# 331658260/Drone-YOLO

Measured on AMD Instinct MI355X. Metric: images/sec @640x640 Drone-YOLO-s, higher is better.
Workload: dtype fp16; 1 GPU; Drone-YOLO-s (yolov8s-p2-repvgg.yaml, nc=10) inference 640x640: layout+forward+decode+NMS, inputs resident in HBM; fp16 storage / fp32 accumulate (BASELINE config 2 names bf16: bf16 storage fails the IoU >= 0.999 bar - 0.995 - so the headline runs the 16-bit format that meets it; same MFMA rate, same bytes); batch_per_gpu=256, global_batch=256, parallelism=batch-split x1, no collective, hipgraph=True, streams=2, max_det=300

## Files before the change

drone-yolo_amd/csrc/conv3x3_hreg.hip:

```cpp
#include "common_hip.h"
#include "conv_args.h"

namespace DY_NS {


struct HregArgs {
  const void* x;
  const void* w;
  const float* bias;
  const void* res;
  void* y;
  int N, H, W, Cin, ldx, Cout, ldy, ldres, act;
  int tilesX, tilesY, tilesN, nSpatial;
  unsigned x_bytes, y_bytes, r_bytes;
  double* stats;
  const float* bnb_mean;
  const float* bnb_rstd;
  const float* bnb_gamma;
  const float* bnb_beta;
  int bnb_act;
  int dbg;
};

#ifdef DYOLO_ABLATE
#define HR_DBG(bit) (p.dbg & (bit))
#else
#define HR_DBG(bit) 0
#endif

constexpr int kHrTH = 8, kHrTW = 16, kHrHH = 10, kHrHW = 24;
constexpr int kHrStage = 16 * 1024;
constexpr int kHrStages = 3;

template <typename T, int NCH, bool RES, bool STATS = false, bool BNB = false, int BW = 3>
__global__ __launch_bounds__(256, NCH <= 2 ? (BNB ? BW : 3) : 2) void conv3x3_hreg_kernel(const HregArgs p) {
  static_assert(!(BNB && (RES || STATS)), "BNB: its own mode");
  constexpr bool SLOTS = STATS || BNB, RLOAD = RES || BNB;
  constexpr int EPC = Elem<T>::EPC;
  __shared__ __attribute__((aligned(1024))) unsigned char smem[kHrStages * kHrStage];
  __shared__ f32x4 bnc[BNB ? 64 : 1];
  const int tid = threadIdx.x, lane = tid & 63, wave = tid >> 6;
  const int lq = lane >> 4, lr = lane & 15;
  const __amdgpu_buffer_rsrc_t yrs = __builtin_amdgcn_make_buffer_rsrc(p.y, 0, p.y_bytes, 0x00020000);
  const __amdgpu_buffer_rsrc_t rrs = __builtin_amdgcn_make_buffer_rsrc(const_cast<void*>(p.res ? p.res : p.y), 0, p.res ? p.r_bytes : 0u, 0x00020000);

  const int G = (int)gridDim.x;
  const int logical = ((int)blockIdx.x & 7) * (G >> 3) + ((int)blockIdx.x >> 3);
  const int nt = logical % p.tilesN;
  const int sb = logical / p.tilesN, Gs = G / p.tilesN;
  const int myTiles = sb < p.nSpatial ? (p.nSpatial - sb + Gs - 1) / Gs : 0;
  if constexpr (SLOTS) {
    if (blockIdx.x == 0)
      for (int i = tid; i < 2 * p.Cout; i += 256) p.stats[i] = 0.0;
    if (myTiles <= 0 && tid < 128) {
      const int co = nt * 64 + (tid & 63);
      if (co < p.Cout) p.stats[(size_t)(1 + sb) * 2 * p.Cout + (tid >> 6) * p.Cout + co] = 0.0;
    }
  }
  if (myTiles <= 0) return;
  const int nItems = myTiles * NCH;

  u32x4 wreg[NCH][9];
  {
    const u32x4* wg = reinterpret_cast<const u32x4*>(p.w) + (size_t)nt * NCH * 9 * 4 * 64;
#pragma unroll
    for (int c = 0; c < NCH; ++c)
#pragma unroll
      for (int t = 0; t < 9; ++t) wreg[c][t] = wg[((c * 9 + t) * 4 + wave) * 64 + lane];
  }
  const f32x4 bias4 = *reinterpret_cast<const f32x4*>(p.bias + nt * 64 + wave * 16 + lq * 4);

  constexpr int NDMA = 4;
  constexpr unsigned kOob = 0xfffffff0u;
  const unsigned pre = (unsigned)((p.W + 1) * p.ldx) * 2u;
  const __amdgpu_buffer_rsrc_t xrs = __builtin_amdgcn_make_buffer_rsrc(const_cast<char*>(reinterpret_cast<const char*>(p.x)) - pre, 0, p.x_bytes + pre, 0x00020000);
  unsigned rel[NDMA];
  int hyx[NDMA];
#pragma unroll
  for (int k = 0; k < NDMA; ++k) {
    const int s = (k * 4 + wave) * 64 + lane;
    const int pix = s >> 2, part = s & 3;
    const int hy = pix / kHrHW, hx = pix - hy * kHrHW;
    const bool dead = hx >= kHrTW + 2 || hy >= kHrHH;
    rel[k] = dead ? kOob : (unsigned)((hy * p.W + hx) * p.ldx + (part ^ ((hx >> 1) & 3)) * EPC) * 2u;
    hyx[k] = hy | (hx << 8);
  }
  unsigned voff[NDMA];
  unsigned l_base = 0;
  int l_tile = sb, l_chunk = 0, l_item = 0;
  auto setup_tile = [&](int tile) {
    const int tx = tile % p.tilesX;
    const int r = tile / p.tilesX;
    const int ty = r % p.tilesY, n = r / p.tilesY;
    const int y0 = ty * kHrTH, x0 = tx * kHrTW;
    l_base = (unsigned)(((n * p.H + y0) * p.W + x0) * p.ldx) * 2u;
    const bool interior = y0 > 0 && y0 + kHrTH + 1 <= p.H && x0 > 0 && x0 + kHrTW + 1 <= p.W;
    if (interior) {
#pragma unroll
      for (int k = 0; k < NDMA; ++k) voff[k] = rel[k];
    } else {
#pragma unroll
      for (int k = 0; k < NDMA; ++k) {
        const int gy = y0 - 1 + (hyx[k] & 255), gx = x0 - 1 + (hyx[k] >> 8);
        voff[k] = ((unsigned)gy < (unsigned)p.H && (unsigned)gx < (unsigned)p.W) ? rel[k] : kOob;
      }
    }
  };
  auto issue_dma = [&](int stage) {
    unsigned char* sa = smem + stage * kHrStage;
    const bool live = l_item < nItems && !(HR_DBG(4) && l_item >= 2);
    if (live) {
      const unsigned soff = l_base + (unsigned)l_chunk * (4u * EPC * (unsigned)sizeof(T));
#pragma unroll
      for (int k = 0; k < NDMA; ++k)
        __builtin_amdgcn_raw_ptr_buffer_load_lds(xrs, (__attribute__((address_space(3))) void*)(sa + (k * 4 + wave) * 1024), 16, (int)voff[k], (int)soff, 0, 0);
      ++l_item;
      if (++l_chunk == NCH) {
        l_chunk = 0;
        l_tile += Gs;
        if (l_item < nItems) setup_tile(l_tile);
      }
    } else {
#pragma unroll
      for (int k = 0; k < NDMA; ++k)
        __builtin_amdgcn_raw_ptr_buffer_load_lds(xrs, (__attribute__((address_space(3))) void*)(sa + (k * 4 + wave) * 1024), 16, (int)kOob, 0, 0, 0);
    }
  };

  int lane_base[3];
#pragma unroll
  for (int q = 0; q < 3; ++q) lane_base[q] = (lr + q) * 64 + ((lq ^ (((lr + q) >> 1) & 3)) * 16);

  f32x4 acc[kHrTH];
#pragma unroll
  for (int o = 0; o < kHrTH; ++o) acc[o] = bias4;

  auto compute = [&](int stg, int c) {
    const unsigned char* sa = smem + stg * kHrStage;
#pragma unroll
    for (int iy = 0; iy < kHrHH; ++iy) {
      u32x4 a[3];
#pragma unroll
      for (int q = 0; q < 3; ++q) a[q] = *reinterpret_cast<const u32x4*>(sa + lane_base[q] + (HR_DBG(8) ? 0 : iy * (kHrHW * 64)));
#pragma unroll
      for (int r = 0; r < 3; ++r) {
        const int o = iy - r;
        if (o >= 0 && o < kHrTH) {
#pragma unroll
          for (int q = 0; q < 3; ++q) {
            if (HR_DBG(2)) asm volatile("" ::"v"(a[q]));
            else acc[o] = Elem<T>::mma(wreg[c][r * 3 + q], a[q], acc[o]);
          }
        }
      }
    }
  };

  typedef __attribute__((ext_vector_type(4))) T t4;
  u32x4 rl[kHrTH / 2];
  auto load_residual = [&](int tile) {
    const int tx = tile % p.tilesX;
    const int r = tile / p.tilesX;
    const int ty = r % p.tilesY, n = r / p.tilesY;
    const int xx = tx * kHrTW + lr;
    const int co16 = nt * 64 + wave * 16 + (lq >> 1) * 8;
#pragma unroll
    for (int o = 0; o < kHrTH; o += 2) {
      const int yy = ty * kHrTH + o + (lq & 1);
      const bool ok = yy < p.H && xx < p.W;
      const unsigned off = ok ? (unsigned)((((size_t)(n * p.H + yy) * p.W + xx) * (size_t)p.ldres + co16) * sizeof(T)) : 0xfffffff0u;
      rl[o / 2] = __builtin_amdgcn_raw_buffer_load_b128(rrs, off, 0, 0);
    }
  };
  unsigned lane_out[kHrTH / 2];
  {
    const int co16 = nt * 64 + wave * 16 + (lq >> 1) * 8;
#pragma unroll
    for (int o = 0; o < kHrTH; o += 2) lane_out[o / 2] = (unsigned)(((o + (lq & 1)) * p.W + lr) * p.ldy + co16) * (unsigned)sizeof(T);
  }
  float st_sum[4] = {0.f, 0.f, 0.f, 0.f}, st_sq[4] = {0.f, 0.f, 0.f, 0.f};
  if constexpr (BNB) {
    if (tid < 64) {
      const int co = nt * 64 + tid;
      const float mu = p.bnb_mean[co], rs = p.bnb_rstd[co], gr = p.bnb_gamma[co] * rs;
      bnc[tid] = f32x4{rs, -mu * rs, gr, p.bnb_beta[co] - gr * mu};
    }
    asm volatile("s_waitcnt lgkmcnt(0)" ::: "memory");
  }
  auto epilogue = [&](int tile) {
    const int tx = tile % p.tilesX;
    const int r = tile / p.tilesX;
    const int ty = r % p.tilesY, n = r / p.tilesY;
    const int y0 = ty * kHrTH, x0 = tx * kHrTW;
    const unsigned out_base = (unsigned)(((n * p.H + y0) * p.W + x0) * p.ldy) * (unsigned)sizeof(T);
    const bool whole = y0 + kHrTH <= p.H && x0 + kHrTW <= p.W;
    u32x2 pk[kHrTH];
#pragma unroll
    for (int o = 0; o < kHrTH; ++o) {
      float v[4] = {acc[o][0], acc[o][1], acc[o][2], acc[o][3]};
      if (p.act == DY_ACT_SILU) {
#pragma unroll
        for (int e = 0; e < 4; ++e) v[e] = silu_f32(v[e]);
      }
      if constexpr (RES) {
        const auto sx = __builtin_amdgcn_permlane16_swap(rl[o / 2][0], rl[o / 2][2], false, false);
        const auto sy = __builtin_amdgcn_permlane16_swap(rl[o / 2][1], rl[o / 2][3], false, false);
        const t4 rr = __builtin_bit_cast(t4, u32x2{sx[o & 1], sy[o & 1]});
#pragma unroll
        for (int e = 0; e < 4; ++e) v[e] += Elem<T>::to_f32(rr[e]);
      }
      t4 ov;
#pragma unroll
      for (int e = 0; e < 4; ++e) ov[e] = Elem<T>::from_f32(v[e]);
      if constexpr (STATS) {
        if (whole || (y0 + o < p.H && x0 + lr < p.W)) {
#pragma unroll
          for (int e = 0; e < 4; ++e) {
            const float f = Elem<T>::to_f32(ov[e]);
            st_sum[e] += f, st_sq[e] += f * f;
          }
        }
      }
      if constexpr (BNB) {
        const auto sx = __builtin_amdgcn_permlane16_swap(rl[o / 2][0], rl[o / 2][2], false, false);
        const auto sy = __builtin_amdgcn_permlane16_swap(rl[o / 2][1], rl[o / 2][3], false, false);
        const t4 zz = __builtin_bit_cast(t4, u32x2{sx[o & 1], sy[o & 1]});
        if (whole || (y0 + o < p.H && x0 + lr < p.W)) {
#pragma unroll
          for (int e = 0; e < 4; ++e) {
            const f32x4 k = bnc[wave * 16 + lq * 4 + e];
            const float zf = Elem<T>::to_f32(zz[e]);
            const float xh = zf * k[0] + k[1];
            float du = Elem<T>::to_f32(ov[e]);
            if (p.bnb_act == DY_ACT_SILU) {
              const float u = zf * k[2] + k[3];
              const float sg = __builtin_amdgcn_rcpf(1.0f + __builtin_amdgcn_exp2f(u * -1.4426950408889634f));
              du *= sg * (1.0f + u * (1.0f - sg));
            }
            st_sum[e] += du, st_sq[e] += du * xh;
          }
        }
      }
      pk[o] = __builtin_bit_cast(u32x2, ov);
      acc[o] = bias4;
    }
#pragma unroll
    for (int o = 0; o < kHrTH; o += 2) {
      const auto sx = __builtin_amdgcn_permlane16_swap(pk[o][0], pk[o + 1][0], false, false);
      const auto sy = __builtin_amdgcn_permlane16_swap(pk[o][1], pk[o + 1][1], false, false);
      unsigned off = lane_out[o / 2];
      if (!whole) off = (y0 + o + (lq & 1) < p.H && x0 + lr < p.W) ? off : kOob;
      __builtin_amdgcn_raw_buffer_store_b128(u32x4{sx[0], sy[0], sx[1], sy[1]}, yrs, HR_DBG(1) ? kOob : off, (int)out_base, 0);
    }
  };

  setup_tile(l_tile);
  issue_dma(0);
  issue_dma(1 % kHrStages);
  asm volatile("s_waitcnt vmcnt(0)" ::: "memory");
  __builtin_amdgcn_s_barrier();
  int c_tile = sb;
  int stage = 0;
  for (int it = 0; it < nItems; it += NCH) {
#pragma unroll
    for (int c = 0; c < NCH; ++c) {
      if constexpr (RLOAD) {
        if (c == NCH - 1) load_residual(c_tile);
      }
      issue_dma(stage + 2 >= kHrStages ? stage + 2 - kHrStages : stage + 2);
      compute(stage, c);
      if (c == NCH - 1) {
        epilogue(c_tile);
        c_tile += Gs;
      }
      asm volatile("s_waitcnt vmcnt(0)" ::: "memory");
      __builtin_amdgcn_s_barrier();
      stage = stage + 1 == kHrStages ? 0 : stage + 1;
    }
  }
  if constexpr (SLOTS) {
#pragma unroll
    for (int e = 0; e < 4; ++e) {
      float a = st_sum[e], b = st_sq[e];
#pragma unroll
      for (int m = 1; m < 16; m <<= 1) a += __shfl_xor(a, m, 64), b += __shfl_xor(b, m, 64);
      const int co = nt * 64 + wave * 16 + lq * 4 + e;
      if (lr == 0 && co < p.Cout) {
        double* slot = p.stats + (size_t)(1 + sb) * 2 * p.Cout;
        slot[co] = (double)a, slot[p.Cout + co] = (double)b;
      }
    }
  }
}

constexpr int kH2TH = 4, kH2TW = 16, kH2HH = 9, kH2Pitch = 40, kH2PlaneB = 24;
constexpr int kH2Stage = 24 * 1024;

template <typename T, int NCH, bool STATS = false>
__global__ __launch_bounds__(256, 2) void conv3x3_hreg_s2_kernel(const HregArgs p) {
  constexpr int EPC = Elem<T>::EPC;
  __shared__ __attribute__((aligned(1024))) unsigned char smem[kHrStages * kH2Stage];
  const int tid = threadIdx.x, lane = tid & 63, wave = tid >> 6;
  const int lq = lane >> 4, lr = lane & 15;
  const __amdgpu_buffer_rsrc_t yrs = __builtin_amdgcn_make_buffer_rsrc(p.y, 0, p.y_bytes, 0x00020000);
  const int Ho = (p.H - 1) / 2 + 1, Wo = (p.W - 1) / 2 + 1;

  const int G = (int)gridDim.x;
  const int logical = ((int)blockIdx.x & 7) * (G >> 3) + ((int)blockIdx.x >> 3);
  const int nt = logical % p.tilesN;
  const int sb = logical / p.tilesN, Gs = G / p.tilesN;
  const int myTiles = sb < p.nSpatial ? (p.nSpatial - sb + Gs - 1) / Gs : 0;
  if constexpr (STATS) {
    if (blockIdx.x == 0)
      for (int i = tid; i < 2 * p.Cout; i += 256) p.stats[i] = 0.0;
    if (myTiles <= 0 && tid < 128) {
      const int co = nt * 64 + (tid & 63);
      if (co < p.Cout) p.stats[(size_t)(1 + sb) * 2 * p.Cout + (tid >> 6) * p.Cout + co] = 0.0;
    }
  }
  if (myTiles <= 0) return;
  const int nItems = myTiles * NCH;

  u32x4 wreg[NCH][9];
  {
    const u32x4* wg = reinterpret_cast<const u32x4*>(p.w) + (size_t)nt * NCH * 9 * 4 * 64;
#pragma unroll
    for (int c = 0; c < NCH; ++c)
#pragma unroll
      for (int t = 0; t < 9; ++t) wreg[c][t] = wg[((c * 9 + t) * 4 + wave) * 64 + lane];
  }
  const f32x4 bias4 = *reinterpret_cast<const f32x4*>(p.bias + nt * 64 + wave * 16 + lq * 4);

  constexpr int NDMA = 6;
  constexpr unsigned kOob = 0xfffffff0u;
  const unsigned pre = (unsigned)((p.W + 1) * p.ldx) * 2u;
  const __amdgpu_buffer_rsrc_t xrs = __builtin_amdgcn_make_buffer_rsrc(const_cast<char*>(reinterpret_cast<const char*>(p.x)) - pre, 0, p.x_bytes + pre, 0x00020000);
  unsigned rel[NDMA];
  int hyx[NDMA];
#pragma unroll
  for (int k = 0; k < NDMA; ++k) {
    const int s = (k * 4 + wave) * 64 + lane;
    const int slot = s >> 2, part = s & 3;
    const int hy = slot / kH2Pitch, c = slot - hy * kH2Pitch;
    const bool planeB = c >= kH2PlaneB;
    const int ci = planeB ? c - kH2PlaneB : c;
    const int hx = planeB ? 2 * ci + 1 : 2 * ci;
    const bool dead = hy >= kH2HH || hx > 2 * kH2TW;
    rel[k] = dead ? kOob : (unsigned)((hy * p.W + hx) * p.ldx + (part ^ ((ci >> 1) & 3)) * EPC) * 2u;
    hyx[k] = hy | (hx << 8);
  }
  unsigned voff[NDMA];
  unsigned l_base = 0;
  int l_tile = sb, l_chunk = 0, l_item = 0;
  auto setup_tile = [&](int tile) {
    const int tx = tile % p.tilesX;
    const int r = tile / p.tilesX;
    const int ty = r % p.tilesY, n = r / p.tilesY;
    const int y0 = 2 * ty * kH2TH, x0 = 2 * tx * kH2TW;
    l_base = (unsigned)(((n * p.H + y0) * p.W + x0) * p.ldx) * 2u;
    const bool interior = y0 > 0 && y0 - 1 + kH2HH <= p.H && x0 > 0 && x0 + 2 * kH2TW <= p.W;
    if (interior) {
#pragma unroll
      for (int k = 0; k < NDMA; ++k) voff[k] = rel[k];
    } else {
#pragma unroll
      for (int k = 0; k < NDMA; ++k) {
        const int gy = y0 - 1 + (hyx[k] & 255), gx = x0 - 1 + (hyx[k] >> 8);
        voff[k] = ((unsigned)gy < (unsigned)p.H && (unsigned)gx < (unsigned)p.W) ? rel[k] : kOob;
      }
    }
  };
  auto issue_dma = [&](int stage) {
    unsigned char* sa = smem + stage * kH2Stage;
    const bool live = l_item < nItems;
    if (live) {
      const unsigned soff = l_base + (unsigned)l_chunk * (4u * EPC * (unsigned)sizeof(T));
#pragma unroll
      for (int k = 0; k < NDMA; ++k)
        __builtin_amdgcn_raw_ptr_buffer_load_lds(xrs, (__attribute__((address_space(3))) void*)(sa + (k * 4 + wave) * 1024), 16, (int)voff[k], (int)soff, 0, 0);
      ++l_item;
      if (++l_chunk == NCH) {
        l_chunk = 0;
        l_tile += Gs;
        if (l_item < nItems) setup_tile(l_tile);
      }
    } else {
#pragma unroll
      for (int k = 0; k < NDMA; ++k)
        __builtin_amdgcn_raw_ptr_buffer_load_lds(xrs, (__attribute__((address_space(3))) void*)(sa + (k * 4 + wave) * 1024), 16, (int)kOob, 0, 0, 0);
    }
  };

  int lane_base[3];
  lane_base[0] = lr * 64 + ((lq ^ ((lr >> 1) & 3)) * 16);
  lane_base[1] = (kH2PlaneB + lr) * 64 + ((lq ^ ((lr >> 1) & 3)) * 16);
  lane_base[2] = (lr + 1) * 64 + ((lq ^ (((lr + 1) >> 1) & 3)) * 16);

  f32x4 acc[kH2TH];
#pragma unroll
  for (int o = 0; o < kH2TH; ++o) acc[o] = bias4;

  auto compute = [&](int stg, int c) {
    const unsigned char* sa = smem + stg * kH2Stage;
#pragma unroll
    for (int iy = 0; iy < kH2HH; ++iy) {
      u32x4 a[3];
#pragma unroll
      for (int q = 0; q < 3; ++q) a[q] = *reinterpret_cast<const u32x4*>(sa + lane_base[q] + iy * (kH2Pitch * 64));
#pragma unroll
      for (int r = 0; r < 3; ++r) {
        if ((iy - r) % 2 == 0) {
          const int o = (iy - r) / 2;
          if (iy - r >= 0 && o < kH2TH) {
#pragma unroll
            for (int q = 0; q < 3; ++q) acc[o] = Elem<T>::mma(wreg[c][r * 3 + q], a[q], acc[o]);
          }
        }
      }
    }
  };

  typedef __attribute__((ext_vector_type(4))) T t4;
  unsigned lane_out[kH2TH / 2];
  {
    const int co16 = nt * 64 + wave * 16 + (lq >> 1) * 8;
#pragma unroll
    for (int o = 0; o < kH2TH; o += 2) lane_out[o / 2] = (unsigned)(((o + (lq & 1)) * Wo + lr) * p.ldy + co16) * (unsigned)sizeof(T);
  }
  float st_sum[4] = {0.f, 0.f, 0.f, 0.f}, st_sq[4] = {0.f, 0.f, 0.f, 0.f};
  auto epilogue = [&](int tile) {
    const int tx = tile % p.tilesX;
    const int r = tile / p.tilesX;
    const int ty = r % p.tilesY, n = r / p.tilesY;
    const int y0 = ty * kH2TH, x0 = tx * kH2TW;
    const unsigned out_base = (unsigned)(((n * Ho + y0) * Wo + x0) * p.ldy) * (unsigned)sizeof(T);
    const bool whole = y0 + kH2TH <= Ho && x0 + kH2TW <= Wo;
    u32x2 pk[kH2TH];
#pragma unroll
    for (int o = 0; o < kH2TH; ++o) {
      float v[4] = {acc[o][0], acc[o][1], acc[o][2], acc[o][3]};
      if (p.act == DY_ACT_SILU) {
#pragma unroll
        for (int e = 0; e < 4; ++e) v[e] = silu_f32(v[e]);
      }
      t4 ov;
#pragma unroll
      for (int e = 0; e < 4; ++e) ov[e] = Elem<T>::from_f32(v[e]);
      pk[o] = __builtin_bit_cast(u32x2, ov);
      if constexpr (STATS) {
        if (whole || (y0 + o < Ho && x0 + lr < Wo)) {
#pragma unroll
          for (int e = 0; e < 4; ++e) {
            const float f = Elem<T>::to_f32(ov[e]);
            st_sum[e] += f, st_sq[e] += f * f;
          }
        }
      }
      acc[o] = bias4;
    }
#pragma unroll
    for (int o = 0; o < kH2TH; o += 2) {
      const auto sx = __builtin_amdgcn_permlane16_swap(pk[o][0], pk[o + 1][0], false, false);
      const auto sy = __builtin_amdgcn_permlane16_swap(pk[o][1], pk[o + 1][1], false, false);
      unsigned off = lane_out[o / 2];
      if (!whole) off = (y0 + o + (lq & 1) < Ho && x0 + lr < Wo) ? off : kOob;
      __builtin_amdgcn_raw_buffer_store_b128(u32x4{sx[0], sy[0], sx[1], sy[1]}, yrs, off, (int)out_base, 0);
    }
  };

  setup_tile(l_tile);
  issue_dma(0);
  issue_dma(1);
  asm volatile("s_waitcnt vmcnt(0)" ::: "memory");
  __builtin_amdgcn_s_barrier();
  int c_tile = sb;
  int stage = 0;
  for (int it = 0; it < nItems; it += NCH) {
#pragma unroll
    for (int c = 0; c < NCH; ++c) {
      issue_dma(stage + 2 >= kHrStages ? stage + 2 - kHrStages : stage + 2);
      compute(stage, c);
      if (c == NCH - 1) {
        epilogue(c_tile);
        c_tile += Gs;
      }
      asm volatile("s_waitcnt vmcnt(0)" ::: "memory");
      __builtin_amdgcn_s_barrier();
      stage = stage + 1 == kHrStages ? 0 : stage + 1;
    }
  }
  if constexpr (STATS) {
#pragma unroll
    for (int e = 0; e < 4; ++e) {
      float a = st_sum[e], b = st_sq[e];
#pragma unroll
      for (int m = 1; m < 16; m <<= 1) a += __shfl_xor(a, m, 64), b += __shfl_xor(b, m, 64);
      const int co = nt * 64 + wave * 16 + lq * 4 + e;
      if (lr == 0 && co < p.Cout) {
        double* slot = p.stats + (size_t)(1 + sb) * 2 * p.Cout;
        slot[co] = (double)a, slot[p.Cout + co] = (double)b;
      }
    }
  }
}

[[maybe_unused]] constexpr int kBnbWgs = 2;
template <typename T>
static int launch_hreg(const HregArgs& a, hipStream_t st) {
  HregArgs p = a;
  const int nch = p.Cin / 32;
  int grid = 256 * (nch <= 2 ? 3 : 2);
  const long long nwork = (long long)p.nSpatial * p.tilesN;
  if (nwork < grid) grid = (int)nwork;
  const int q = 8 * p.tilesN;
  grid = (grid + q - 1) / q * q;
  const bool res = p.res != nullptr;
#ifndef DYOLO_L2E_BUILD
  if (p.bnb_mean) {
    static const int bw = dy_ablate("DYOLO_BNB_WGS") ? dy_ablate("DYOLO_BNB_WGS") : kBnbWgs;
    if (nch == 2 && bw == 2) {
      int g2 = 256 * 2;
      if (nwork < g2) g2 = (int)nwork;
      grid = (g2 + q - 1) / q * q;
      hipLaunchKernelGGL((conv3x3_hreg_kernel<T, 2, false, false, true, 2>), dim3((unsigned)grid), dim3(256), 0, st, p);
    } else if (nch == 2) {
      hipLaunchKernelGGL((conv3x3_hreg_kernel<T, 2, false, false, true, 3>), dim3((unsigned)grid), dim3(256), 0, st, p);
    } else {
      hipLaunchKernelGGL((conv3x3_hreg_kernel<T, 4, false, false, true>), dim3((unsigned)grid), dim3(256), 0, st, p);
    }
    note_stats(grid / p.tilesN);
    return check_launch("conv3x3_hreg_kernel<bnb>");
  }
#endif
  if (p.stats) {
    if (nch == 1) hipLaunchKernelGGL((conv3x3_hreg_kernel<T, 1, false, true>), dim3((unsigned)grid), dim3(256), 0, st, p);
    else if (nch == 2) hipLaunchKernelGGL((conv3x3_hreg_kernel<T, 2, false, true>), dim3((unsigned)grid), dim3(256), 0, st, p);
    else hipLaunchKernelGGL((conv3x3_hreg_kernel<T, 4, false, true>), dim3((unsigned)grid), dim3(256), 0, st, p);
    note_stats(grid / p.tilesN);
    return check_launch("conv3x3_hreg_kernel");
  }
  if (nch == 1) {
    if (res) hipLaunchKernelGGL((conv3x3_hreg_kernel<T, 1, true>), dim3((unsigned)grid), dim3(256), 0, st, p);
    else hipLaunchKernelGGL((conv3x3_hreg_kernel<T, 1, false>), dim3((unsigned)grid), dim3(256), 0, st, p);
  } else if (nch == 2) {
    if (res) hipLaunchKernelGGL((conv3x3_hreg_kernel<T, 2, true>), dim3((unsigned)grid), dim3(256), 0, st, p);
    else hipLaunchKernelGGL((conv3x3_hreg_kernel<T, 2, false>), dim3((unsigned)grid), dim3(256), 0, st, p);
  } else {
    hipLaunchKernelGGL((conv3x3_hreg_kernel<T, 4, false>), dim3((unsigned)grid), dim3(256), 0, st, p);
  }
  return check_launch("conv3x3_hreg_kernel");
}

template <typename T>
static int launch_hreg_s2(const HregArgs& a, hipStream_t st) {
  HregArgs p = a;
  int grid = 256 * 2;
  const long long nwork = (long long)p.nSpatial * p.tilesN;
  if (nwork < grid) grid = (int)nwork;
  const int q = 8 * p.tilesN;
  grid = (grid + q - 1) / q * q;
#ifndef DYOLO_L2E_BUILD
  if (p.stats) {
    hipLaunchKernelGGL((conv3x3_hreg_s2_kernel<T, 2, true>), dim3((unsigned)grid), dim3(256), 0, st, p);
    note_stats(grid / p.tilesN);
    return check_launch("conv3x3_hreg_s2_kernel");
  }
#endif
  hipLaunchKernelGGL((conv3x3_hreg_s2_kernel<T, 2>), dim3((unsigned)grid), dim3(256), 0, st, p);
  return check_launch("conv3x3_hreg_s2_kernel");
}

int conv3x3_hreg_try(const dy_conv_desc* d, hipStream_t st) {
  static const int off = dy_ablate("DYOLO_NO_HREG");
  if (off) return 1;
  if (!(d->dtype == DY_BF16 || d->dtype == DY_F16) || d->out_f32 || d->ksize != 3 || d->pad != 1 || d->groups > 1 || d->up2x || d->x2) return 1;
  if (d->stride == 2) {
    if (d->cin != 64 || d->cout % 64 != 0 || d->cout > 256 || d->residual) return 1;
    const long long xb2 = (long long)d->batch * d->h * d->w_in * d->ld_x * 2, yb2 = (long long)d->batch * d->ho * d->wo * d->ld_y * 2;
    if (xb2 >= (1ll << 31) || yb2 >= (1ll << 32) - 64 || d->ld_y % 8 || (reinterpret_cast<uintptr_t>(d->y) & 15)) return 1;
    HregArgs a{};
    a.x = d->x, a.w = d->w, a.bias = d->bias, a.res = nullptr, a.y = d->y;
    a.N = d->batch, a.H = d->h, a.W = d->w_in, a.Cin = d->cin, a.ldx = d->ld_x, a.Cout = d->cout, a.ldy = d->ld_y, a.ldres = 0, a.act = d->act;
    a.tilesX = (d->wo + kH2TW - 1) / kH2TW;
    a.tilesY = (d->ho + kH2TH - 1) / kH2TH;
    a.tilesN = d->cout / 64;
    a.nSpatial = d->batch * a.tilesY * a.tilesX;
    a.x_bytes = (unsigned)xb2, a.y_bytes = (unsigned)yb2, a.r_bytes = 0;
    a.stats = (d->y_dtype1 || d->bnb_z) ? nullptr : d->bn_stats;
    return d->dtype == DY_BF16 ? launch_hreg_s2<bf16_t>(a, st) : launch_hreg_s2<f16_t>(a, st);
  }
  if (d->stride != 1) return 1;
  if ((d->cin != 64 && d->cin != 128) || d->cout % 64 != 0 || d->cout > 256 || d->residual) return 1;
  if (d->ho != d->h || d->wo != d->w_in) return 1;
  const long long xb = (long long)d->batch * d->h * d->w_in * d->ld_x * 2, yb = (long long)d->batch * d->ho * d->wo * d->ld_y * 2;
  const long long rb = d->residual ? (long long)d->batch * d->ho * d->wo * d->ld_res * 2 : 0;
  if (xb >= (1ll << 31) || yb >= (1ll << 32) - 64 || rb >= (1ll << 32) - 64) return 1;
  if (d->ld_y % 8 || (reinterpret_cast<uintptr_t>(d->y) & 15) || (d->residual && (d->ld_res % 8 || (reinterpret_cast<uintptr_t>(d->residual) & 15)))) return 1;
  HregArgs a{};
  a.x = d->x, a.w = d->w, a.bias = d->bias, a.res = d->residual, a.y = d->y;
  a.N = d->batch, a.H = d->h, a.W = d->w_in, a.Cin = d->cin, a.ldx = d->ld_x, a.Cout = d->cout, a.ldy = d->ld_y, a.ldres = d->ld_res, a.act = d->act;
  a.tilesX = (d->wo + kHrTW - 1) / kHrTW;
  a.tilesY = (d->ho + kHrTH - 1) / kHrTH;
  a.tilesN = d->cout / 64;
  a.nSpatial = d->batch * a.tilesY * a.tilesX;
  a.x_bytes = (unsigned)xb, a.y_bytes = (unsigned)yb, a.r_bytes = (unsigned)rb;
  a.stats = d->bn_stats;
  if (d->bnb_z) {
    const long long zb = (long long)d->batch * d->ho * d->wo * d->bnb_ld_z * 2;
#ifdef DYOLO_L2E_BUILD
    const bool built = false;
#else
    const bool built = d->bn_stats && !d->y_dtype1 && d->act == DY_ACT_NONE && d->cin != 32 && zb < (1ll << 32) - 64 && d->bnb_ld_z % 8 == 0 && (reinterpret_cast<uintptr_t>(d->bnb_z) & 15) == 0;
#endif
    if (built) {
      a.res = d->bnb_z, a.ldres = d->bnb_ld_z, a.r_bytes = (unsigned)zb;
      a.bnb_mean = d->bnb_mean, a.bnb_rstd = d->bnb_rstd, a.bnb_gamma = d->bnb_gamma, a.bnb_beta = d->bnb_beta, a.bnb_act = d->bnb_act;
    } else {
      a.stats = nullptr;
    }
  }
  a.dbg = dy_ablate("DYOLO_DBG");
  return d->dtype == DY_BF16 ? launch_hreg<bf16_t>(a, st) : launch_hreg<f16_t>(a, st);
}

}
```

Measured before the change: 20270 images/sec.

## Stage residual through the LDS DMA pipeline in the 3x3 hreg conv

The stride-1 3x3 register-weight conv now accepts a residual input (cin=cout=64, no stats or BN fusion). The residual tile is fetched with buffer-load-to-LDS as an extra pipeline item after the input-channel chunks, and the epilogue reads it from shared memory instead of doing per-lane global loads plus permlane swaps. The aim is to route residual layers to this kernel and overlap the residual fetch with compute, at the cost of one more pipeline step per tile and a narrower residual size limit.

```diff
diff --git a/drone-yolo_amd/csrc/conv3x3_hreg.hip b/drone-yolo_amd/csrc/conv3x3_hreg.hip
--- a/drone-yolo_amd/csrc/conv3x3_hreg.hip
+++ b/drone-yolo_amd/csrc/conv3x3_hreg.hip
@@ -35,7 +35,9 @@
 template <typename T, int NCH, bool RES, bool STATS = false, bool BNB = false, int BW = 3>
 __global__ __launch_bounds__(256, NCH <= 2 ? (BNB ? BW : 3) : 2) void conv3x3_hreg_kernel(const HregArgs p) {
   static_assert(!(BNB && (RES || STATS)), "BNB: its own mode");
-  constexpr bool SLOTS = STATS || BNB, RLOAD = RES || BNB;
+  static_assert(!(RES && STATS), "the staged residual has no statistics form");
+  constexpr bool SLOTS = STATS || BNB;
+  constexpr int NI = NCH + (RES ? 1 : 0);
   constexpr int EPC = Elem<T>::EPC;
   __shared__ __attribute__((aligned(1024))) unsigned char smem[kHrStages * kHrStage];
   __shared__ f32x4 bnc[BNB ? 64 : 1];
@@ -58,7 +60,7 @@
     }
   }
   if (myTiles <= 0) return;
-  const int nItems = myTiles * NCH;
+  const int nItems = myTiles * NI;
 
   u32x4 wreg[NCH][9];
   {
@@ -88,12 +90,16 @@
   unsigned voff[NDMA];
   unsigned l_base = 0;
   int l_tile = sb, l_chunk = 0, l_item = 0;
+  [[maybe_unused]] const unsigned r_step = (unsigned)(2 * p.W * p.ldres) * 2u;
+  [[maybe_unused]] unsigned l_rbase = 0;
+  [[maybe_unused]] int l_y0 = 0, l_x0 = 0;
   auto setup_tile = [&](int tile) {
     const int tx = tile % p.tilesX;
     const int r = tile / p.tilesX;
     const int ty = r % p.tilesY, n = r / p.tilesY;
     const int y0 = ty * kHrTH, x0 = tx * kHrTW;
     l_base = (unsigned)(((n * p.H + y0) * p.W + x0) * p.ldx) * 2u;
+    if constexpr (RES) l_rbase = (unsigned)(((n * p.H + y0) * p.W + x0) * p.ldres) * 2u, l_y0 = y0, l_x0 = x0;
     const bool interior = y0 > 0 && y0 + kHrTH + 1 <= p.H && x0 > 0 && x0 + kHrTW + 1 <= p.W;
     if (interior) {
 #pragma unroll
@@ -101,7 +107,15 @@
     } else {
 #pragma unroll
       for (int k = 0; k < NDMA; ++k) {
-        const int gy = y0 - 1 + (hyx[k] & 255), gx = x0 - 1 + (hyx[k] >> 8);
+        int hv = hyx[k];
+        if constexpr (RES) {
+          int t = tid;
+          asm volatile("" : "+v"(t));
+          const int pix = (k * 4 + (t >> 6)) * 16 + ((t >> 2) & 15);
+          const int hy = pix / kHrHW;
+          hv = hy | ((pix - hy * kHrHW) << 8);
+        }
+        const int gy = y0 - 1 + (hv & 255), gx = x0 - 1 + (hv >> 8);
         voff[k] = ((unsigned)gy < (unsigned)p.H && (unsigned)gx < (unsigned)p.W) ? rel[k] : kOob;
       }
     }
@@ -110,12 +124,26 @@
     unsigned char* sa = smem + stage * kHrStage;
     const bool live = l_item < nItems && !(HR_DBG(4) && l_item >= 2);
     if (live) {
-      const unsigned soff = l_base + (unsigned)l_chunk * (4u * EPC * (unsigned)sizeof(T));
-#pragma unroll
-      for (int k = 0; k < NDMA; ++k)
-        __builtin_amdgcn_raw_ptr_buffer_load_lds(xrs, (__attribute__((address_space(3))) void*)(sa + (k * 4 + wave) * 1024), 16, (int)voff[k], (int)soff, 0, 0);
+      if (RES && l_chunk == NCH) {
+        const bool whole = l_y0 + kHrTH <= p.H && l_x0 + kHrTW <= p.W;
+        int t = tid;
+        asm volatile("" : "+v"(t));
+        const int px = t & 15;
+        const unsigned r_rel0 = (unsigned)((((wave >> 1) * p.W + px) * p.ldres + nt * 64 + ((wave & 1) * 2 + ((t >> 5) & 1)) * 16 + ((t >> 4) & 1) * 8) * 2);
+#pragma unroll
+        for (int k = 0; k < NDMA; ++k) {
+          unsigned off = r_rel0 + (unsigned)k * r_step;
+          if (!whole) off = (l_y0 + 2 * k + (wave >> 1) < p.H && l_x0 + px < p.W) ? off : kOob;
+          __builtin_amdgcn_raw_ptr_buffer_load_lds(rrs, (__attribute__((address_space(3))) void*)(sa + (k * 4 + wave) * 1024), 16, (int)off, (int)l_rbase, 0, 0);
+        }
+      } else {
+        const unsigned soff = l_base + (unsigned)l_chunk * (4u * EPC * (unsigned)sizeof(T));
+#pragma unroll
+        for (int k = 0; k < NDMA; ++k)
+          __builtin_amdgcn_raw_ptr_buffer_load_lds(xrs, (__attribute__((address_space(3))) void*)(sa + (k * 4 + wave) * 1024), 16, (int)voff[k], (int)soff, 0, 0);
+      }
       ++l_item;
-      if (++l_chunk == NCH) {
+      if (++l_chunk == NI) {
         l_chunk = 0;
         l_tile += Gs;
         if (l_item < nItems) setup_tile(l_tile);
@@ -187,7 +215,7 @@
     }
     asm volatile("s_waitcnt lgkmcnt(0)" ::: "memory");
   }
-  auto epilogue = [&](int tile) {
+  auto epilogue = [&](int tile, [[maybe_unused]] int stg) {
     const int tx = tile % p.tilesX;
     const int r = tile / p.tilesX;
     const int ty = r % p.tilesY, n = r / p.tilesY;
@@ -195,6 +223,12 @@
     const unsigned out_base = (unsigned)(((n * p.H + y0) * p.W + x0) * p.ldy) * (unsigned)sizeof(T);
     const bool whole = y0 + kHrTH <= p.H && x0 + kHrTW <= p.W;
     u32x2 pk[kHrTH];
+    [[maybe_unused]] int res_lane = 0;
+    if constexpr (RES) {
+      int t = tid;
+      asm volatile("" : "+v"(t));
+      res_lane = stg * kHrStage + ((t >> 6) * 32 + ((t >> 5) & 1) * 16 + (t & 15)) * 16 + ((t >> 4) & 1) * 8;
+    }
 #pragma unroll
     for (int o = 0; o < kHrTH; ++o) {
       float v[4] = {acc[o][0], acc[o][1], acc[o][2], acc[o][3]};
@@ -203,9 +237,7 @@
         for (int e = 0; e < 4; ++e) v[e] = silu_f32(v[e]);
       }
       if constexpr (RES) {
-        const auto sx = __builtin_amdgcn_permlane16_swap(rl[o / 2][0], rl[o / 2][2], false, false);
-        const auto sy = __builtin_amdgcn_permlane16_swap(rl[o / 2][1], rl[o / 2][3], false, false);
-        const t4 rr = __builtin_bit_cast(t4, u32x2{sx[o & 1], sy[o & 1]});
+        const t4 rr = *reinterpret_cast<const t4*>(smem + res_lane + o * (4 * 512));
 #pragma unroll
         for (int e = 0; e < 4; ++e) v[e] += Elem<T>::to_f32(rr[e]);
       }
@@ -248,7 +280,7 @@
     for (int o = 0; o < kHrTH; o += 2) {
       const auto sx = __builtin_amdgcn_permlane16_swap(pk[o][0], pk[o + 1][0], false, false);
       const auto sy = __builtin_amdgcn_permlane16_swap(pk[o][1], pk[o + 1][1], false, false);
-      unsigned off = lane_out[o / 2];
+      unsigned off = RES ? lane_out[0] + (unsigned)(o * p.W * p.ldy) * (unsigned)sizeof(T) : lane_out[o / 2];
       if (!whole) off = (y0 + o + (lq & 1) < p.H && x0 + lr < p.W) ? off : kOob;
       __builtin_amdgcn_raw_buffer_store_b128(u32x4{sx[0], sy[0], sx[1], sy[1]}, yrs, HR_DBG(1) ? kOob : off, (int)out_base, 0);
     }
@@ -261,16 +293,16 @@
   __builtin_amdgcn_s_barrier();
   int c_tile = sb;
   int stage = 0;
-  for (int it = 0; it < nItems; it += NCH) {
-#pragma unroll
-    for (int c = 0; c < NCH; ++c) {
-      if constexpr (RLOAD) {
+  for (int it = 0; it < nItems; it += NI) {
+#pragma unroll
+    for (int c = 0; c < NI; ++c) {
+      if constexpr (BNB) {
         if (c == NCH - 1) load_residual(c_tile);
       }
       issue_dma(stage + 2 >= kHrStages ? stage + 2 - kHrStages : stage + 2);
-      compute(stage, c);
-      if (c == NCH - 1) {
-        epilogue(c_tile);
+      if (c < NCH) compute(stage, c);
+      if (c == NI - 1) {
+        epilogue(c_tile, stage);
         c_tile += Gs;
       }
       asm volatile("s_waitcnt vmcnt(0)" ::: "memory");
@@ -540,8 +572,7 @@
     return check_launch("conv3x3_hreg_kernel");
   }
   if (nch == 1) {
-    if (res) hipLaunchKernelGGL((conv3x3_hreg_kernel<T, 1, true>), dim3((unsigned)grid), dim3(256), 0, st, p);
-    else hipLaunchKernelGGL((conv3x3_hreg_kernel<T, 1, false>), dim3((unsigned)grid), dim3(256), 0, st, p);
+    hipLaunchKernelGGL((conv3x3_hreg_kernel<T, 1, false>), dim3((unsigned)grid), dim3(256), 0, st, p);
   } else if (nch == 2) {
     if (res) hipLaunchKernelGGL((conv3x3_hreg_kernel<T, 2, true>), dim3((unsigned)grid), dim3(256), 0, st, p);
     else hipLaunchKernelGGL((conv3x3_hreg_kernel<T, 2, false>), dim3((unsigned)grid), dim3(256), 0, st, p);
@@ -590,11 +621,12 @@
     return d->dtype == DY_BF16 ? launch_hreg_s2<bf16_t>(a, st) : launch_hreg_s2<f16_t>(a, st);
   }
   if (d->stride != 1) return 1;
-  if ((d->cin != 64 && d->cin != 128) || d->cout % 64 != 0 || d->cout > 256 || d->residual) return 1;
+  if ((d->cin != 64 && d->cin != 128) || d->cout % 64 != 0 || d->cout > 256) return 1;
+  if (d->residual && (d->cin != 64 || d->cout != 64 || d->bn_stats || d->bnb_z)) return 1;
   if (d->ho != d->h || d->wo != d->w_in) return 1;
   const long long xb = (long long)d->batch * d->h * d->w_in * d->ld_x * 2, yb = (long long)d->batch * d->ho * d->wo * d->ld_y * 2;
   const long long rb = d->residual ? (long long)d->batch * d->ho * d->wo * d->ld_res * 2 : 0;
-  if (xb >= (1ll << 31) || yb >= (1ll << 32) - 64 || rb >= (1ll << 32) - 64) return 1;
+  if (xb >= (1ll << 31) || yb >= (1ll << 32) - 64 || rb >= (1ll << 31)) return 1;
   if (d->ld_y % 8 || (reinterpret_cast<uintptr_t>(d->y) & 15) || (d->residual && (d->ld_res % 8 || (reinterpret_cast<uintptr_t>(d->residual) & 15)))) return 1;
   HregArgs a{};
   a.x = d->x, a.w = d->w, a.bias = d->bias, a.res = d->residual, a.y = d->y;
```

After: 20340 images/sec, median of 6. Within noise of the previous version (+0.3%).
